# shenyunhang/NA-fWebSOD

Measured on AMD Instinct MI355X. Metric: images/sec (600px, 2000 proposals) VGG16-C5 WSDDN fwd+bwd, higher is better.
Workload: dtype f32 (2xf16 split, 3-pass f16 MFMA, fp32 accumulate)

## Files before the change

na-fwebsod_amd/csrc/misc_ops.hip:

```cpp
#include <float.h>
#include <math.h>
#include "naws_common.h"

thread_local int g_naws_last_hip_error = 0;

extern "C" const char* naws_version(void) { return "naws-hip 0.1 (gfx950)"; }
extern "C" int naws_last_hip_error(void) { return g_naws_last_hip_error; }

#include <atomic>
#include <mutex>
#include <string.h>
namespace {
constexpr int LDS_SLOTS = 512;
constexpr int MAX_DEV = 256;
struct LdsSlot {
  std::atomic<const void*> kernel;
  std::atomic<unsigned long long> dev[MAX_DEV / 64];
};
LdsSlot g_lds_slots[LDS_SLOTS];
std::mutex g_lds_mutex;
std::atomic<int> g_knobs[NAWS_KNOB_COUNT] = {{0}, {0}, {0}, {11}, {0}, {42}, {0}, {0}, {0}};
const char* const g_knob_names[NAWS_KNOB_COUNT] = {"gemm", "x3", "h2", "conv_ring", "conv_bn",
                                                    "roi_nw", "wino", "split", "sgd_wgs"};
}

int naws_allow_lds_impl(const void* kernel, int bytes) {
  int dev = 0;
  if (hipGetDevice(&dev) != hipSuccess) return naws_check_launch();
  const bool in_range = dev >= 0 && dev < MAX_DEV;
  const size_t h0 = ((uintptr_t)kernel >> 4) % LDS_SLOTS;
  if (in_range) {
    size_t h = h0;
    for (int probe = 0; probe < LDS_SLOTS; ++probe, h = (h + 1) % LDS_SLOTS) {
      const void* k = g_lds_slots[h].kernel.load(std::memory_order_acquire);
      if (k == kernel) {
        if ((g_lds_slots[h].dev[dev >> 6].load(std::memory_order_acquire) >> (dev & 63)) & 1ULL)
          return NAWS_OK;
        break;
      }
      if (k == nullptr) break;
    }
  }
  std::lock_guard<std::mutex> lock(g_lds_mutex);
  LdsSlot* slot = nullptr;
  if (in_range) {
    size_t h = h0;
    for (int probe = 0; probe < LDS_SLOTS; ++probe, h = (h + 1) % LDS_SLOTS) {
      const void* k = g_lds_slots[h].kernel.load(std::memory_order_relaxed);
      if (k == kernel) { slot = &g_lds_slots[h]; break; }
      if (k == nullptr) {
        slot = &g_lds_slots[h];
        slot->kernel.store(kernel, std::memory_order_release);
        break;
      }
    }
  }
// ... 676 lines not shown
```

na-fwebsod_amd/csrc/naws_common.h:

```cpp
#pragma once
#include <hip/hip_runtime.h>
#include <stdint.h>
#include <algorithm>
#include "naws.h"

#define NAWS_WAVE 64

extern thread_local int g_naws_last_hip_error;

static inline int naws_check_launch() {
  hipError_t e = hipGetLastError();
  if (e != hipSuccess) {
    g_naws_last_hip_error = (int)e;
    return NAWS_ERR_LAUNCH;
  }
  return NAWS_OK;
}

int naws_allow_lds_impl(const void* kernel, int bytes);
template <typename K>
static inline int naws_allow_lds(K kernel, int bytes = 160 * 1024) {
  return naws_allow_lds_impl(reinterpret_cast<const void*>(kernel), bytes);
}

int naws_wino_col_gemm_impl(int P, int Cout, int Cin, const void* V2, const float* invV,
                            const void* U2, const float* scaleU, float* S, hipStream_t stream);

enum NawsKnob { NAWS_KNOB_GEMM = 0, NAWS_KNOB_X3, NAWS_KNOB_H2, NAWS_KNOB_CONV_RING,
                NAWS_KNOB_CONV_BN, NAWS_KNOB_ROI_NW, NAWS_KNOB_WINO, NAWS_KNOB_SPLIT, NAWS_KNOB_SGD_WGS,
                NAWS_KNOB_COUNT };
int naws_knob(int knob);

#define NAWS_REQUIRE_PTR(p) \
  do {                      \
    if ((p) == nullptr) return NAWS_ERR_NULL; \
  } while (0)

static inline int64_t naws_cdiv(int64_t a, int64_t b) { return (a + b - 1) / b; }

__device__ __forceinline__ float wave_sum(float v) {
#pragma unroll
  for (int o = 32; o > 0; o >>= 1) v += __shfl_xor(v, o, 64);
  return v;
}
__device__ __forceinline__ float wave_max(float v) {
#pragma unroll
  for (int o = 32; o > 0; o >>= 1) v = fmaxf(v, __shfl_xor(v, o, 64));
  return v;
}

__device__ __host__ __forceinline__ uint32_t naws_hash_u32(uint64_t seed, uint64_t idx) {
  uint64_t z = seed + 0x9E3779B97F4A7C15ull * (idx + 1);
  z = (z ^ (z >> 30)) * 0xBF58476D1CE4E5B9ull;
  z = (z ^ (z >> 27)) * 0x94D049BB133111EBull;
  z = z ^ (z >> 31);
  return (uint32_t)(z >> 40);
}
__device__ __host__ __forceinline__ bool naws_keep(uint64_t seed, uint64_t idx, uint32_t thr24) {
  return naws_hash_u32(seed, idx) >= thr24;
}
static inline uint32_t naws_drop_threshold(float ratio) {
  double t = (double)ratio * 16777216.0;
  if (t < 0) t = 0;
// ... 174 lines not shown
```

na-fwebsod_amd/csrc/roi_ops.hip:

```cpp
#include <float.h>
#include <stdlib.h>
#include "naws_common.h"

namespace {

struct RoiBins {
  int batch, start_w, start_h, roi_w, roi_h;
};

__device__ __forceinline__ RoiBins roi_frame(const float* roi, float spatial_scale) {
  RoiBins b;
  b.batch = (int)roi[0];
  int start_w = (int)roundf(roi[1] * spatial_scale);
  int start_h = (int)roundf(roi[2] * spatial_scale);
  int end_w = (int)roundf(roi[3] * spatial_scale);
  int end_h = (int)roundf(roi[4] * spatial_scale);
  b.start_w = start_w;
  b.start_h = start_h;
  b.roi_w = max(end_w - start_w + 1, 1);
  b.roi_h = max(end_h - start_h + 1, 1);
  return b;
}

__device__ __forceinline__ void bin_range(int p, float bin_size, int roi_start, int limit,
// ... 116 lines not shown
          }
          for (; w < we; ++w) {
            const float4 v = *reinterpret_cast<const float4*>(row + (int64_t)w * C);
            NAWS_UPD(v)
          }
#undef NAWS_UPD
        }
      }
      tile[(0 * 64 + lane) * PW + pw] = best.x * scale;
      tile[(1 * 64 + lane) * PW + pw] = best.y * scale;
      tile[(2 * 64 + lane) * PW + pw] = best.z * scale;
      tile[(3 * 64 + lane) * PW + pw] = best.w * scale;
    }
    __syncthreads();
    const int count = nch * PW;
    for (int i = lane; i < count; i += 64) {
      const int cl = i / PW, pw = i - cl * PW;
      Y[obase + (int64_t)cl * nb + ph * PW + pw] = tile[((cl & 3) * 64 + (cl >> 2)) * PW + pw];
    }
    __syncthreads();
  }
}

struct RoiPlaneOut {
  unsigned short* P;
  float* inv_scale;
  const unsigned* amax_words;
  int n_words;
  long long plane;
  int R;
  int bf16;
};

template <bool PLANES, bool HIER = false, int NW = 1, int RG = 1>
__global__ __launch_bounds__(64 * NW) void roi_pool_nhwc_xcd_kernel(
    const float* __restrict__ X, int C, int H, int W, const float* __restrict__ rois, int R,
    const float* __restrict__ boost, int PH, int PW, float spatial_scale, int nslices,
    float* __restrict__ Y, RoiPlaneOut po, const float* __restrict__ M2 = nullptr,
    const float* __restrict__ M4 = nullptr) {
  static_assert(NW % RG == 0, "waves per roi");
  extern __shared__ __attribute__((aligned(16))) char smem_raw[];
  const int nb = PH * PW;
  float* tiles = reinterpret_cast<float*>(smem_raw);
  float* s_scale = tiles + RG * 64 * nb;
  const int slice = blockIdx.x % nslices;
  const int r0 = (blockIdx.x / nslices) * RG;
  const int lane = threadIdx.x & 63;
  const int wave = threadIdx.x >> 6;
  const int q = wave % RG;
  const int r = r0 + q;
  const int cg = lane & 15, g = lane >> 4;
  const int c0 = slice * 64;
  float* tile = tiles + q * 64 * nb;

  if (r < R) {
    const RoiBins rb = roi_frame(rois + (int64_t)r * 5, spatial_scale);
    const float bin_h = (float)rb.roi_h / (float)PH;
    const float bin_w = (float)rb.roi_w / (float)PW;
    const float scale = boost ? boost[r] : 1.0f;
    const int64_t img_off = (int64_t)rb.batch * H * W * C + c0 + cg * 4;
    const float* Xn = X + img_off;
    if constexpr (PLANES) {
      if (wave < RG && lane == 0 && !po.bf16) {
        const float bound =
            __uint_as_float(po.amax_words[min(rb.batch, po.n_words - 1)]) * fabsf(scale);
        float sc, isc;
        naws_f16x2_scales(__float_as_uint(bound), sc, isc);
        s_scale[q] = sc;
        if (slice == 0) po.inv_scale[r] = isc;
      }
    }

    const int pwg = (PW + 3) / 4;
    for (int step = wave / RG; step < PH * pwg; step += NW / RG) {
      const int ph = step / pwg, pw0 = (step - ph * pwg) * 4;
      int hs, he;
      bin_range(ph, bin_h, rb.start_h, H, hs, he);
      const int pw = pw0 + g;
      const bool lane_on = pw < PW;
      int ws = 0, we = 0;
      if (lane_on) bin_range(pw, bin_w, rb.start_w, W, ws, we);
      const bool empty = (he <= hs) || (we <= ws);
      const float init = empty ? 0.0f : -FLT_MAX;
      float4 best = make_float4(init, init, init, init);
#define NAWS_UPD(v) \
  best.x = (v.x > best.x) ? v.x : best.x; best.y = (v.y > best.y) ? v.y : best.y; \
  best.z = (v.z > best.z) ? v.z : best.z; best.w = (v.w > best.w) ? v.w : best.w;
      int hbeg = hs;
      if constexpr (HIER) {
        const int dmin = min(he - hs, we - ws);
        if (dmin >= 2) {
          const int Lb = dmin >= 4 ? 4 : 2;
          const float* S = (dmin >= 4 ? M4 : M2) + img_off;
          const int hl = he - Lb, wl = we - Lb;
          for (int h = hs; h < he; h += 2 * Lb) {
            const float* q0 = S + (int64_t)min(h, hl) * W * C;
            const float* q1 = S + (int64_t)min(h + Lb, hl) * W * C;
            int w = ws;
            for (; w + 2 * Lb < we; w += 2 * Lb) {
              const float4 a0 = *reinterpret_cast<const float4*>(q0 + (int64_t)w * C);
              const float4 a1 = *reinterpret_cast<const float4*>(q0 + (int64_t)(w + Lb) * C);
              const float4 b0 = *reinterpret_cast<const float4*>(q1 + (int64_t)w * C);
              const float4 b1 = *reinterpret_cast<const float4*>(q1 + (int64_t)(w + Lb) * C);
              NAWS_UPD(a0) NAWS_UPD(a1) NAWS_UPD(b0) NAWS_UPD(b1)
            }
            {
              const int w0 = min(w, wl), w1 = min(w + Lb, wl);
              const float4 a0 = *reinterpret_cast<const float4*>(q0 + (int64_t)w0 * C);
              const float4 a1 = *reinterpret_cast<const float4*>(q0 + (int64_t)w1 * C);
              const float4 b0 = *reinterpret_cast<const float4*>(q1 + (int64_t)w0 * C);
              const float4 b1 = *reinterpret_cast<const float4*>(q1 + (int64_t)w1 * C);
              NAWS_UPD(a0) NAWS_UPD(a1) NAWS_UPD(b0) NAWS_UPD(b1)
            }
// ... 20 lines not shown
        }
        for (; w < we; ++w) {
          const float4 a = *reinterpret_cast<const float4*>(q0 + (int64_t)w * C);
          const float4 b = *reinterpret_cast<const float4*>(q1 + (int64_t)w * C);
          NAWS_UPD(a) NAWS_UPD(b)
        }
      }
      for (; h < he; ++h) {
        const float* row = Xn + (int64_t)h * W * C;
        int w = ws;
        for (; w + 4 <= we; w += 4) {
          const float4 v0 = *reinterpret_cast<const float4*>(row + (int64_t)(w + 0) * C);
          const float4 v1 = *reinterpret_cast<const float4*>(row + (int64_t)(w + 1) * C);
          const float4 v2 = *reinterpret_cast<const float4*>(row + (int64_t)(w + 2) * C);
          const float4 v3 = *reinterpret_cast<const float4*>(row + (int64_t)(w + 3) * C);
          NAWS_UPD(v0) NAWS_UPD(v1) NAWS_UPD(v2) NAWS_UPD(v3)
        }
        for (; w < we; ++w) {
          const float4 v = *reinterpret_cast<const float4*>(row + (int64_t)w * C);
          NAWS_UPD(v)
        }
      }
#undef NAWS_UPD
      if (lane_on) {
        const int bin = ph * PW + pw;
        tile[(cg * 4 + 0) * nb + bin] = best.x * scale;
        tile[(cg * 4 + 1) * nb + bin] = best.y * scale;
        tile[(cg * 4 + 2) * nb + bin] = best.z * scale;
        tile[(cg * 4 + 3) * nb + bin] = best.w * scale;
      }
    }
  }
  __syncthreads();
  const int count = 64 * nb;
  if constexpr (!PLANES) {
    for (int i = threadIdx.x; i < RG * count; i += 64 * NW) {
      const int qq = i / count, k = i - qq * count;
      if (r0 + qq < R) Y[((int64_t)(r0 + qq) * C + c0) * nb + k] = tiles[i];
    }
  } else {
    const int slab0 = slice * (count / 16);
    for (int i = threadIdx.x; i < RG * (count / 8); i += 64 * NW) {
      const int hh = i & 1, qq = (i >> 1) % RG, j = i / (2 * RG);
      if (r0 + qq >= R) continue;
      const float* src = tiles + qq * count + j * 16 + hh * 8;
      if (po.bf16) {
        unsigned short q8[8];
#pragma unroll
        for (int e = 0; e < 8; ++e) {
          const __bf16 b = (__bf16)src[e];
          q8[e] = *reinterpret_cast<const unsigned short*>(&b);
        }
        uint4 w;
        w.x = q8[0] | ((unsigned)q8[1] << 16); w.y = q8[2] | ((unsigned)q8[3] << 16);
        w.z = q8[4] | ((unsigned)q8[5] << 16); w.w = q8[6] | ((unsigned)q8[7] << 16);
        *reinterpret_cast<uint4*>(po.P + ((long long)(slab0 + j) * po.R + r0 + qq) * 16 + hh * 8) = w;
        continue;
      }
      const float sc = s_scale[qq];
      unsigned short hi[8], lo[8];
#pragma unroll
      for (int e = 0; e < 8; ++e) {
        const float t = src[e] * sc;
        const _Float16 a = (_Float16)t;
        float rr = t - (float)a;
        if (!(fabsf(t) <= 65504.f)) rr = 0.f;
        const _Float16 b = (_Float16)rr;
        hi[e] = *reinterpret_cast<const unsigned short*>(&a);
        lo[e] = *reinterpret_cast<const unsigned short*>(&b);
      }
      const long long dst = ((long long)(slab0 + j) * po.R + r0 + qq) * 16 + hh * 8;
      uint4 wh, wl;
      wh.x = hi[0] | ((unsigned)hi[1] << 16); wh.y = hi[2] | ((unsigned)hi[3] << 16);
      wh.z = hi[4] | ((unsigned)hi[5] << 16); wh.w = hi[6] | ((unsigned)hi[7] << 16);
// ... 28 lines not shown
  if (k >= K) return;
  const int sl = threadIdx.x >> 4, kk = threadIdx.x & 15;
  unsigned w[8];
#pragma unroll
  for (int i = 0; i < 8; ++i) w[i] = t[sl][2 * i][kk] | ((unsigned)t[sl][2 * i + 1][kk] << 16);
  unsigned short* o = dst + ((long long)blockIdx.y * K + k) * 16;
  *reinterpret_cast<uint4*>(o) = make_uint4(w[0], w[1], w[2], w[3]);
  *reinterpret_cast<uint4*>(o + 8) = make_uint4(w[4], w[5], w[6], w[7]);
}

template <int STEP>
__global__ __launch_bounds__(256) void roi_maxmap_kernel(const float* __restrict__ S, int H, int W,
                                                         int C, float* __restrict__ D,
                                                         long long total4) {
  const long long i = (long long)blockIdx.x * 256 + threadIdx.x;
  if (i >= total4) return;
  const int c4 = C / 4;
  const int cq = (int)(i % c4);
  const long long pix = i / c4;
  const int x = (int)(pix % W), y = (int)((pix / W) % H);
  const int dy = (y + STEP < H) ? STEP : 0, dx = (x + STEP < W) ? STEP : 0;
  const float* base = S + (pix * C + cq * 4);
  const float4 v00 = *reinterpret_cast<const float4*>(base);
  const float4 v01 = *reinterpret_cast<const float4*>(base + (long long)dx * C);
  const float4 v10 = *reinterpret_cast<const float4*>(base + (long long)dy * W * C);
  const float4 v11 = *reinterpret_cast<const float4*>(base + ((long long)dy * W + dx) * C);
  float4 m = make_float4(-FLT_MAX, -FLT_MAX, -FLT_MAX, -FLT_MAX);
#define NAWS_MX(b, v) \
  b.x = (v.x > b.x) ? v.x : b.x; b.y = (v.y > b.y) ? v.y : b.y; \
  b.z = (v.z > b.z) ? v.z : b.z; b.w = (v.w > b.w) ? v.w : b.w;
  NAWS_MX(m, v00) NAWS_MX(m, v01) NAWS_MX(m, v10) NAWS_MX(m, v11)
#undef NAWS_MX
  *reinterpret_cast<float4*>(D + (pix * C + cq * 4)) = m;
}

__global__ void roi_pool_nchw_kernel(int64_t total, const float* __restrict__ X, int C, int H,
                                     int W, const float* __restrict__ rois,
                                     const float* __restrict__ boost, int PH, int PW,
                                     float spatial_scale, float* __restrict__ Y,
                                     int32_t* __restrict__ argmax) {
  for (int64_t idx = (int64_t)blockIdx.x * blockDim.x + threadIdx.x; idx < total;
       idx += (int64_t)gridDim.x * blockDim.x) {
    int pw = (int)(idx % PW);
    int ph = (int)((idx / PW) % PH);
    int c = (int)((idx / PW / PH) % C);
    int r = (int)(idx / PW / PH / C);
    const RoiBins rb = roi_frame(rois + (int64_t)r * 5, spatial_scale);
    const float bin_h = (float)rb.roi_h / (float)PH;
    const float bin_w = (float)rb.roi_w / (float)PW;
    int hs, he, ws, we;
    bin_range(ph, bin_h, rb.start_h, H, hs, he);
    bin_range(pw, bin_w, rb.start_w, W, ws, we);
    const bool empty = (he <= hs) || (we <= ws);
    float best = empty ? 0.0f : -FLT_MAX;
    int besti = -1;
    const float* Xc = X + ((int64_t)rb.batch * C + c) * H * W;
    for (int h = hs; h < he; ++h)
      for (int w = ws; w < we; ++w) {
        float v = Xc[h * W + w];
        if (v > best) { best = v; besti = h * W + w; }
      }
    Y[idx] = best * (boost ? boost[r] : 1.0f);
    if (argmax) argmax[idx] = besti;
  }
}

// ... 76 lines not shown
                       rois, boost, pooled_h, pooled_w, spatial_scale, Y, argmax);
  }
  return naws_check_launch();
}

extern "C" int naws_roi_pool_f_f16x2_fwd(const float* X, int N, int C, int H, int W,
                                         const float* rois, int R, const float* boost,
                                         int pooled_h, int pooled_w, float spatial_scale,
                                         const uint32_t* amax_words, int n_words, void* planes,
                                         float* scales, void* stream) {
  if (R <= 0 || N <= 0 || C <= 0 || H <= 0 || W <= 0 || pooled_h <= 0 || pooled_w <= 0 || n_words <= 0)
    return NAWS_ERR_SHAPE;
  NAWS_REQUIRE_PTR(X); NAWS_REQUIRE_PTR(rois); NAWS_REQUIRE_PTR(amax_words);
  NAWS_REQUIRE_PTR(planes); NAWS_REQUIRE_PTR(scales);
  const long long K = (long long)C * pooled_h * pooled_w;
  if (C % 64 != 0 || pooled_h * pooled_w > 256 || K % 32 != 0 || (int64_t)R * (C / 64) >= 0x7fffffffLL)
    return NAWS_ERR_UNSUPPORTED;
  if ((((uintptr_t)X | (uintptr_t)planes) & 15) != 0) return NAWS_ERR_ARG;
  RoiPlaneOut po;
  po.P = (unsigned short*)planes; po.inv_scale = scales + R; po.amax_words = (const unsigned*)amax_words;
  po.n_words = n_words; po.plane = K * R; po.R = R; po.bf16 = 0;
  hipLaunchKernelGGL(roi_pool_nhwc_xcd_kernel<true>, dim3((unsigned)(R * (C / 64))), dim3(64),
                     (size_t)(64 * pooled_h * pooled_w + 1) * sizeof(float), (hipStream_t)stream, X, C,
                     H, W, rois, R, boost, pooled_h, pooled_w, spatial_scale, C / 64, (float*)nullptr,
                     po);
  return naws_check_launch();
}

extern "C" int64_t naws_roi_pool_workspace_floats(int N, int C, int H, int W) {
  if (N <= 0 || C <= 0 || H <= 0 || W <= 0) return 0;
  return (int64_t)2 * N * H * W * C;
}

static int roi_maxmaps(const float* X, int N, int C, int H, int W, float* M2, float* M4,
                       hipStream_t s) {
  const long long total4 = (long long)N * H * W * (C / 4);
  if (naws_cdiv(total4, 256) > 0x7fffffffLL) return NAWS_ERR_UNSUPPORTED;
  hipLaunchKernelGGL(roi_maxmap_kernel<1>, dim3((unsigned)naws_cdiv(total4, 256)), dim3(256), 0, s, X, H,
                     W, C, M2, total4);
  hipLaunchKernelGGL(roi_maxmap_kernel<2>, dim3((unsigned)naws_cdiv(total4, 256)), dim3(256), 0, s,
                     (const float*)M2, H, W, C, M4, total4);
  return naws_check_launch();
}

extern "C" int naws_roi_pool_f_nhwc_hier_fwd(const float* X, int N, int C, int H, int W,
                                             const float* rois, int R, const float* boost,
                                             int pooled_h, int pooled_w, float spatial_scale,
                                             float* workspace, float* Y, void* stream) {
  if (R < 0 || N <= 0 || C <= 0 || H <= 0 || W <= 0 || pooled_h <= 0 || pooled_w <= 0)
    return NAWS_ERR_SHAPE;
  if (R == 0) return NAWS_OK;
  NAWS_REQUIRE_PTR(X); NAWS_REQUIRE_PTR(rois); NAWS_REQUIRE_PTR(Y); NAWS_REQUIRE_PTR(workspace);
  if (C % 64 != 0 || pooled_h * pooled_w > 256 || (int64_t)R * (C / 64) >= 0x7fffffffLL)
    return NAWS_ERR_UNSUPPORTED;
  if ((((uintptr_t)X | (uintptr_t)workspace) & 15) != 0) return NAWS_ERR_ARG;
  hipStream_t s = (hipStream_t)stream;
  const int rc = roi_maxmaps(X, N, C, H, W, workspace, workspace + (long long)N * H * W * C, s);
  if (rc != NAWS_OK) return rc;
  hipLaunchKernelGGL((roi_pool_nhwc_xcd_kernel<false, true, 4>), dim3((unsigned)(R * (C / 64))), dim3(256),
                     (size_t)(64 * pooled_h * pooled_w + 1) * sizeof(float), s, X, C, H, W, rois, R,
                     boost, pooled_h, pooled_w, spatial_scale, C / 64, Y, RoiPlaneOut{},
                     (const float*)workspace, (const float*)(workspace + (long long)N * H * W * C));
  return naws_check_launch();
}

static int roi_pool_planes_mapped(const float* X, int N, int C, int H, int W, const float* rois,
                                  int R, const float* boost, int pooled_h, int pooled_w,
                                  float spatial_scale, const uint32_t* amax_words, int n_words,
                                  const float* M2, const float* M4, void* planes, float* scales,
                                  hipStream_t s, int bf16 = 0, int R_total = 0, int r_first = 0) {
  const long long K = (long long)C * pooled_h * pooled_w;
  if (R_total <= 0) { R_total = R; r_first = 0; }
  rois += (long long)r_first * 5;
  if (boost) boost += r_first;
  RoiPlaneOut po;
  po.P = (unsigned short*)planes + (long long)r_first * 16;
  po.inv_scale = scales ? scales + R_total + r_first : nullptr;
  po.amax_words = (const unsigned*)amax_words;
  po.n_words = n_words; po.plane = K * R_total; po.R = R_total; po.bf16 = bf16;
  const int nw = naws_knob(NAWS_KNOB_ROI_NW);
  (void)nw;
#define NAWS_ROI_LAUNCH(NWV, RGV)                                                                    \
  hipLaunchKernelGGL((roi_pool_nhwc_xcd_kernel<true, true, NWV, RGV>),                               \
                     dim3((unsigned)(naws_cdiv(R, RGV) * (C / 64))), dim3(64 * NWV),                  \
                     (size_t)(RGV * 64 * pooled_h * pooled_w + RGV) * sizeof(float), s, X, C, H, W,  \
                     rois, R, boost, pooled_h, pooled_w, spatial_scale, C / 64, (float*)nullptr, po, \
                     M2, M4)
#ifdef NAWS_AB
  if (nw == 41) NAWS_ROI_LAUNCH(4, 1);
  else if (nw == 44) NAWS_ROI_LAUNCH(4, 4);
  else if (nw == 82) NAWS_ROI_LAUNCH(8, 2);
  else if (nw == 84) NAWS_ROI_LAUNCH(8, 4);
  else
#endif
  NAWS_ROI_LAUNCH(4, 2);
#undef NAWS_ROI_LAUNCH
  return naws_check_launch();
}

static int roi_pool_planes_check(const float* X, int N, int C, int H, int W, const float* rois, int R,
                                 int pooled_h, int pooled_w, const uint32_t* amax_words, int n_words,
                                 const void* planes, const float* scales) {
  if (R <= 0 || N <= 0 || C <= 0 || H <= 0 || W <= 0 || pooled_h <= 0 || pooled_w <= 0 || n_words <= 0)
    return NAWS_ERR_SHAPE;
  NAWS_REQUIRE_PTR(X); NAWS_REQUIRE_PTR(rois); NAWS_REQUIRE_PTR(amax_words);
  NAWS_REQUIRE_PTR(planes); NAWS_REQUIRE_PTR(scales);
  const long long K = (long long)C * pooled_h * pooled_w;
  if (C % 64 != 0 || pooled_h * pooled_w > 256 || K % 32 != 0 || (int64_t)R * (C / 64) >= 0x7fffffffLL)
    return NAWS_ERR_UNSUPPORTED;
  if ((((uintptr_t)X | (uintptr_t)planes) & 15) != 0) return NAWS_ERR_ARG;
  return NAWS_OK;
}

extern "C" int naws_roi_pool_f_f16x2_hier_fwd(const float* X, int N, int C, int H, int W,
                                              const float* rois, int R, const float* boost,
                                              int pooled_h, int pooled_w, float spatial_scale,
                                              const uint32_t* amax_words, int n_words,
                                              float* workspace, void* planes, float* scales,
                                              void* stream) {
  int rc = roi_pool_planes_check(X, N, C, H, W, rois, R, pooled_h, pooled_w, amax_words, n_words,
                                 planes, scales);
  if (rc != NAWS_OK) return rc;
  NAWS_REQUIRE_PTR(workspace);
  if (((uintptr_t)workspace & 15) != 0) return NAWS_ERR_ARG;
  hipStream_t s = (hipStream_t)stream;
  float* M4 = workspace + (long long)N * H * W * C;
  rc = roi_maxmaps(X, N, C, H, W, workspace, M4, s);
  if (rc != NAWS_OK) return rc;
// ... 357 lines not shown
```

na-fwebsod_amd/naws_hip/lib.py:

```python
import ctypes as C
import os

_HERE = os.path.dirname(os.path.abspath(__file__))
LIB_PATH = os.environ.get('NAWS_LIB') or os.path.join(os.path.dirname(_HERE), 'lib',
                                                       'libnaws_hip.so')
_ENV_KNOBS = {'NAWS_GEMM_VARIANT': 'gemm', 'NAWS_X3_VARIANT': 'x3', 'NAWS_H2_VARIANT': 'h2',
              'NAWS_CONV_RING': 'conv_ring', 'NAWS_CONV_BN': 'conv_bn', 'NAWS_ROI_NW': 'roi_nw',
              'NAWS_WINO_VARIANT': 'wino', 'NAWS_SPLIT': 'split', 'NAWS_SGD_WGS': 'sgd_wgs'}

OK, ERR_SHAPE, ERR_ARG, ERR_NULL, ERR_LAUNCH, ERR_UNSUPPORTED = 0, -1, -2, -3, -4, -5
_ERR_NAMES = {
    ERR_SHAPE: 'NAWS_ERR_SHAPE', ERR_ARG: 'NAWS_ERR_ARG', ERR_NULL: 'NAWS_ERR_NULL',
    ERR_LAUNCH: 'NAWS_ERR_LAUNCH', ERR_UNSUPPORTED: 'NAWS_ERR_UNSUPPORTED',
}
LAYOUT_NCHW, LAYOUT_NHWC = 0, 1
EPI_NONE, EPI_BIAS, EPI_BIAS_RELU, EPI_BIAS_RELU_DROP, EPI_GATE_POS = range(5)
UN_LOG, UN_SCALE, UN_REPLACE_NAN, UN_LEAKY_RELU, UN_CLIP, UN_RELU = range(6)
BIN_ADD, BIN_SUB, BIN_MUL, BIN_DIV, BIN_GATE_POS = range(5)
PLANES_F16X2, PLANES_BF16X3, PLANES_BF16 = range(3)

p, i32, i64, u64, f32 = C.c_void_p, C.c_int, C.c_int64, C.c_uint64, C.c_float

PROTOTYPES = {
    'naws_conv3x3_c3_nchw_to_nhwc_fwd': [p, p, p, i32, i32, i32, i32, i32, p, p],
    'naws_conv3x3_pack_weight': [p, i32, i32, p, p],
    'naws_conv3x3_nhwc_fwd': [p, p, p, i32, i32, i32, i32, i32, i32, i32, p, p],
    'naws_maxpool2x2_nhwc_fwd': [p, i32, i32, i32, i32, i32, p, p],
    'naws_winograd_weight_transform': [p, i32, i32, p, p],
    'naws_conv3x3_winograd_nhwc_fwd': [p, p, p, i32, i32, i32, i32, i32, i32, i32, p, p, p],
    'naws_nchw_to_nhwc': [p, i32, i32, i32, i32, p, p],
    'naws_nhwc_to_nchw': [p, i32, i32, i32, i32, p, p],
    'naws_roi_pool_f_fwd': [p, i32, i32, i32, i32, i32, p, i32, p, i32, i32, f32, p, p, p],
    'naws_roi_context_fwd': [p, i32, f32, i32, i32, p, p, p],
    'naws_roi_loop_pool_fwd': [p, i32, i32, i32, i32, i32, p, i32, p, i32, i32, f32, p, p, p],
    'naws_roi_feature_boost_fwd': [p, p, i32, i32, p, p],
    'naws_roi_feature_boost_bwd': [p, p, i32, i32, p, p],
    'naws_roi_iou_fwd': [p, i32, p, p],
    'naws_gemm_f32': [i32, i32, i32, i32, i32, p, i32, p, i32, p, i32, i32, i64, i64, i64,
                      i32, p, i64, p, i32, f32, f32, u64, i32, p],
    'naws_dropout_mask': [u64, f32, i64, p, p],
    'naws_colsum_f32': [p, i32, i32, i32, p, i32, p],
# ... 81 lines not shown
    'naws_conv3x3_winograd_nhwc_f16x2_fwd': [p, p, p, p, i32, i32, i32, i32, i32, i32, i32, p, p, p, p, p],
    'naws_winograd4_weight_transform': [p, i32, i32, p, p],
    'naws_conv3x3_winograd4_nhwc_f16x2_fwd': [p, p, p, p, i32, i32, i32, i32, i32, i32, i32, p, p, p, p, p],
    'naws_gemm_f32_f16x2_nt_amax': [i32, i32, i32, p, i64, i64, p, p, i64, i64, p, p, i32, i32,
                                    i64, i64, i64, i64, i64, i32, p, i64, p, i32, f32, f32, u64, i32,
                                    p, i32, p, p, p],
    'naws_gemm_f32_f16x2_nt_cols': [i32, i32, i32, p, i64, i64, p, p, i64, i64, p, p, i32, i32, p, f32,
                                    u64, p, i32, p, i32, i32, p],
    'naws_gemm_f32_amax': [i32, i32, i32, i32, i32, p, i32, p, i32, p, i32, i32, i64, i64, i64,
                           i32, p, i64, p, i32, f32, f32, u64, i32, p, i32, p, p, p],
    'naws_split_f16x2_dual': [p, i32, i32, i32, i32, i64, p, p, p, p, p, i32, p, p, i32, p],
    'naws_gemm_f32_f16x2_nt': [i32, i32, i32, p, i64, i64, p, p, i64, i64, p, p, i32, i32,
                               i64, i64, i64, i64, i64, i32, p, i64, p, i32, f32, f32, u64, i32, p],
}
SPECIAL = {
    'naws_version': ([], C.c_char_p),
    'naws_last_hip_error': ([], i32),
    'naws_entropy_gate_workspace_floats': ([i32, i32, i32, i32], i64),
    'naws_winograd_workspace_floats': ([i32, i32, i32, i32, i32, i32], i64),
    'naws_nms_workspace_bytes': ([i32, i32], i64),
    'naws_roi_label_workspace_bytes': ([i32, i32, i32], i64),
    'naws_softmax_with_loss_n_workspace_floats': ([i32], i64),
    'naws_center_loss_workspace_bytes': ([i32, i32, i32], i64),
    'naws_roi_pool_workspace_floats': ([i32, i32, i32, i32], i64),
    'naws_winograd_f32x3_workspace_floats': ([i32, i32, i32, i32, i32, i32], i64),
    'naws_winograd_f16x2_workspace_floats': ([i32, i32, i32, i32, i32, i32], i64),
    'naws_winograd4_f16x2_workspace_floats': ([i32, i32, i32, i32, i32, i32], i64),
    'naws_gemm_f32_splitk_workspace_floats': ([i32, i32, i32, i32], i64),
}
ALL_SYMBOLS = sorted(list(PROTOTYPES) + list(SPECIAL))
AB_PROTOTYPES = {
    'naws_conv3x3_winograd_nhwc_f16x2_col_fwd': [p, p, p, p, i32, i32, i32, i32, i32, i32, i32, p, p, p,
                                                 p, p],
}


class NawsError(RuntimeError):

    def __init__(self, fn, code, hip_error=0):
        self.fn, self.code, self.hip_error = fn, code, hip_error
        msg = '%s failed: %s' % (fn, _ERR_NAMES.get(code, code))
        if code == ERR_LAUNCH:
            msg += ' (hipError %d)' % hip_error
        super(NawsError, self).__init__(msg)


_lib = None


def load():
    global _lib
    if _lib is not None:
        return _lib
    import torch
    if not os.path.exists(LIB_PATH):
        raise ImportError(
            'libnaws_hip.so not found at %s — build it with `make -C na-fwebsod_amd/csrc` '
            '(or __graft_entry__.build()); there is no CPU fallback.' % LIB_PATH)
    lib = C.CDLL(LIB_PATH)
    for name, argtypes in PROTOTYPES.items():
        fn = getattr(lib, name)
        fn.argtypes, fn.restype = argtypes, i32
    for name, (argtypes, restype) in SPECIAL.items():
        fn = getattr(lib, name)
        fn.argtypes, fn.restype = argtypes, restype
    for name, argtypes in AB_PROTOTYPES.items():
# ... 21 lines not shown
```

na-fwebsod_amd/naws_hip/ops.py:

```python
import ctypes as C

import numpy as np
import torch

from . import lib as L

_f32 = torch.float32


def _stream():
    return torch.cuda.current_stream().cuda_stream


def _chk(t, name, dtype=_f32):
    if not isinstance(t, torch.Tensor) or not t.is_cuda:
        raise TypeError('%s must be a HIP device tensor (the naws ops have no CPU path)' % name)
    if t.dtype != dtype:
        raise TypeError('%s must be %s, got %s' % (name, dtype, t.dtype))
    if not t.is_contiguous():
        raise ValueError('%s must be contiguous' % name)
    return t


def _ptr(t):
# ... 129 lines not shown

def roi_loop_pool(x, rois9, pooled_h=7, pooled_w=7, spatial_scale=0.125, boost=None,
                  layout='NCHW', with_argmax=False):
    _chk(x, 'x'); _chk(rois9, 'rois9')
    if rois9.dim() != 2 or rois9.shape[1] != 9:
        raise L.NawsError('naws_roi_loop_pool_fwd', L.ERR_SHAPE)
    if layout == 'NCHW':
        n, c, h, w = x.shape
        lay = L.LAYOUT_NCHW
    elif layout == 'NHWC':
        n, h, w, c = x.shape
        lay = L.LAYOUT_NHWC
    else:
        raise L.NawsError('naws_roi_loop_pool_fwd', L.ERR_ARG)
    r = rois9.shape[0]
    if boost is not None:
        _chk(boost, 'boost')
        assert boost.numel() == r
    y = torch.empty((r, c, pooled_h, pooled_w), device=x.device, dtype=_f32)
    am = torch.empty((r, c, pooled_h, pooled_w), device=x.device, dtype=torch.int32) \
        if with_argmax else None
    L.call('naws_roi_loop_pool_fwd', x.data_ptr(), lay, n, c, h, w, rois9.data_ptr(), r,
           _ptr(boost), pooled_h, pooled_w, float(spatial_scale), y.data_ptr(), _ptr(am), _stream())
    return (y, am) if with_argmax else y


def roi_maxmaps(x, m2, m4):
    _chk(x, 'x'); _chk(m2, 'm2'); _chk(m4, 'm4')
    if m2.shape != x.shape or m4.shape != x.shape or not (x.is_contiguous() and m2.is_contiguous()
                                                          and m4.is_contiguous()):
        raise TypeError('roi_maxmaps: contiguous maps of x\'s shape')
    n, h, w, c = x.shape
    L.call('naws_roi_maxmaps_fwd', x.data_ptr(), n, c, h, w, m2.data_ptr(), m4.data_ptr(), _stream())


def roi_pool_operand(r, k, device):
    return F16x2(torch.empty((2, k // 16, r, 16), device=device, dtype=torch.float16),
                 torch.empty((2, r), device=device, dtype=_f32))


def roi_pool_f_f16x2_range(x, rois, amax_words, out, r0, r1, maps, pooled_h=7, pooled_w=7,
                           spatial_scale=0.125, boost=None):
    _chk(x, 'x'); _chk(rois, 'rois')
    n, h, w, c = x.shape
    r = rois.shape[0]
    m2, m4 = maps
    _chk(m2, 'm2'); _chk(m4, 'm4')
    if boost is not None:
        _chk(boost, 'boost')
        assert boost.numel() == r
    if out.planes.shape != (2, c * pooled_h * pooled_w // 16, r, 16) or m2.shape != x.shape:
        raise L.NawsError('naws_roi_pool_f_f16x2_mapped_range_fwd', L.ERR_SHAPE)
    L.call('naws_roi_pool_f_f16x2_mapped_range_fwd', x.data_ptr(), n, c, h, w, rois.data_ptr(), r,
           int(r0), int(r1 - r0), _ptr(boost), pooled_h, pooled_w, float(spatial_scale),
           amax_words.data_ptr(), amax_words.numel(), m2.data_ptr(), m4.data_ptr(),
           out.planes.data_ptr(), out.scales.data_ptr(), _stream())
    return out


def roi_pool_f_f16x2(x, rois, amax_words, pooled_h=7, pooled_w=7, spatial_scale=0.125, boost=None,
                     hier=True, maps=None):
    _chk(x, 'x'); _chk(rois, 'rois')
    if rois.dim() != 2 or rois.shape[1] != 5:
        raise L.NawsError('naws_roi_pool_f_f16x2_fwd', L.ERR_SHAPE)
    n, h, w, c = x.shape
    r = rois.shape[0]
# ... 1236 lines not shown
```

Measured before the change: 159.9.

## Fuse ROI max-map passes into one LDS-tiled kernel and reorder slice blocks

Replaces the two elementwise max-map launches with a single tiled kernel that loads an input tile with halo into LDS and writes both the 2x2 and the dilated max maps. This removes one launch and the re-read of M2 from global memory. The ROI pool kernel also gains a block-to-slice mapping that interleaves 8 channel slices per round for cache locality. Behind A/B knobs it adds narrower channel slices and a 4-wide store path. The tiled kernel uses a sizeable LDS allocation, which may limit occupancy.

```diff
diff --git a/na-fwebsod_amd/csrc/misc_ops.hip b/na-fwebsod_amd/csrc/misc_ops.hip
--- a/na-fwebsod_amd/csrc/misc_ops.hip
+++ b/na-fwebsod_amd/csrc/misc_ops.hip
@@ -19,9 +19,11 @@
 };
 LdsSlot g_lds_slots[LDS_SLOTS];
 std::mutex g_lds_mutex;
-std::atomic<int> g_knobs[NAWS_KNOB_COUNT] = {{0}, {0}, {0}, {11}, {0}, {42}, {0}, {0}, {0}};
+std::atomic<int> g_knobs[NAWS_KNOB_COUNT] = {{0}, {0}, {0}, {11}, {0}, {42}, {0}, {0}, {0},
+                                           {0}, {0}};
 const char* const g_knob_names[NAWS_KNOB_COUNT] = {"gemm", "x3", "h2", "conv_ring", "conv_bn",
-                                                    "roi_nw", "wino", "split", "sgd_wgs"};
+                                                    "roi_nw", "wino", "split", "sgd_wgs",
+                                                    "roi_cs", "roi_maps"};
 }
 
 int naws_allow_lds_impl(const void* kernel, int bytes) {
diff --git a/na-fwebsod_amd/csrc/naws_common.h b/na-fwebsod_amd/csrc/naws_common.h
--- a/na-fwebsod_amd/csrc/naws_common.h
+++ b/na-fwebsod_amd/csrc/naws_common.h
@@ -28,7 +28,7 @@
 
 enum NawsKnob { NAWS_KNOB_GEMM = 0, NAWS_KNOB_X3, NAWS_KNOB_H2, NAWS_KNOB_CONV_RING,
                 NAWS_KNOB_CONV_BN, NAWS_KNOB_ROI_NW, NAWS_KNOB_WINO, NAWS_KNOB_SPLIT, NAWS_KNOB_SGD_WGS,
-                NAWS_KNOB_COUNT };
+                NAWS_KNOB_ROI_CS, NAWS_KNOB_ROI_MAPS, NAWS_KNOB_COUNT };
 int naws_knob(int knob);
 
 #define NAWS_REQUIRE_PTR(p) \
diff --git a/na-fwebsod_amd/csrc/roi_ops.hip b/na-fwebsod_amd/csrc/roi_ops.hip
--- a/na-fwebsod_amd/csrc/roi_ops.hip
+++ b/na-fwebsod_amd/csrc/roi_ops.hip
@@ -172,7 +172,7 @@
   int bf16;
 };
 
-template <bool PLANES, bool HIER = false, int NW = 1, int RG = 1>
+template <bool PLANES, bool HIER = false, int NW = 1, int RG = 1, int CS = 64, bool ST2 = false>
 __global__ __launch_bounds__(64 * NW) void roi_pool_nhwc_xcd_kernel(
     const float* __restrict__ X, int C, int H, int W, const float* __restrict__ rois, int R,
     const float* __restrict__ boost, int PH, int PW, float spatial_scale, int nslices,
@@ -181,17 +181,35 @@
   static_assert(NW % RG == 0, "waves per roi");
   extern __shared__ __attribute__((aligned(16))) char smem_raw[];
   const int nb = PH * PW;
+  static_assert(CS == 64 || CS == 32 || CS == 16, "slice width");
+  constexpr int QL = CS / 4;
+  constexpr int SLOTS = 256 / CS;
   float* tiles = reinterpret_cast<float*>(smem_raw);
-  float* s_scale = tiles + RG * 64 * nb;
-  const int slice = blockIdx.x % nslices;
-  const int r0 = (blockIdx.x / nslices) * RG;
+  float* s_scale = tiles + RG * CS * nb;
+  int slice, group;
+  {
+    const int ngroups = (int)(gridDim.x / (unsigned)nslices);
+    const int full = nslices / 8;
+    const int per_round = full ? 8 * ngroups : 0;
+    const int round = full ? (int)(blockIdx.x / (unsigned)per_round) : 0;
+    if (round < full) {
+      const int l = (int)blockIdx.x - round * per_round;
+      slice = round * 8 + (l & 7);
+      group = l >> 3;
+    } else {
+      const int l = (int)blockIdx.x - full * per_round, rem = nslices - full * 8;
+      slice = full * 8 + l % rem;
+      group = l / rem;
+    }
+  }
+  const int r0 = group * RG;
   const int lane = threadIdx.x & 63;
   const int wave = threadIdx.x >> 6;
   const int q = wave % RG;
   const int r = r0 + q;
-  const int cg = lane & 15, g = lane >> 4;
-  const int c0 = slice * 64;
-  float* tile = tiles + q * 64 * nb;
+  const int cg = lane % QL, g = lane / QL;
+  const int c0 = slice * CS;
+  float* tile = tiles + q * CS * nb;
 
   if (r < R) {
     const RoiBins rb = roi_frame(rois + (int64_t)r * 5, spatial_scale);
@@ -212,13 +230,22 @@
     }
 
     const int pwg = (PW + 3) / 4;
-    for (int step = wave / RG; step < PH * pwg; step += NW / RG) {
-      const int ph = step / pwg, pw0 = (step - ph * pwg) * 4;
-      int hs, he;
-      bin_range(ph, bin_h, rb.start_h, H, hs, he);
-      const int pw = pw0 + g;
-      const bool lane_on = pw < PW;
-      int ws = 0, we = 0;
+    const int nsteps = CS == 64 ? PH * pwg : (nb + SLOTS - 1) / SLOTS;
+    for (int step = wave / RG; step < nsteps; step += NW / RG) {
+      int ph, pw, hs = 0, he = 0, ws = 0, we = 0;
+      bool lane_on;
+      if constexpr (CS == 64) {
+        ph = step / pwg;
+        pw = (step - ph * pwg) * 4 + g;
+        lane_on = pw < PW;
+        bin_range(ph, bin_h, rb.start_h, H, hs, he);
+      } else {
+        const int bin = step * SLOTS + g;
+        lane_on = bin < nb;
+        ph = bin / PW;
+        pw = bin - ph * PW;
+        if (lane_on) bin_range(ph, bin_h, rb.start_h, H, hs, he);
+      }
       if (lane_on) bin_range(pw, bin_w, rb.start_w, W, ws, we);
       const bool empty = (he <= hs) || (we <= ws);
       const float init = empty ? 0.0f : -FLT_MAX;
@@ -305,7 +332,7 @@
     }
   }
   __syncthreads();
-  const int count = 64 * nb;
+  const int count = CS * nb;
   if constexpr (!PLANES) {
     for (int i = threadIdx.x; i < RG * count; i += 64 * NW) {
       const int qq = i / count, k = i - qq * count;
@@ -313,6 +340,41 @@
     }
   } else {
     const int slab0 = slice * (count / 16);
+    if constexpr (ST2) {
+      for (int i = threadIdx.x; i < RG * (count / 4); i += 64 * NW) {
+        const int u = i & 3, qq = (i >> 2) % RG, j = i / (4 * RG);
+        if (r0 + qq >= R) continue;
+        const float4 v = *reinterpret_cast<const float4*>(tiles + qq * count + j * 16 + u * 4);
+        const float src[4] = {v.x, v.y, v.z, v.w};
+        const long long dst = ((long long)(slab0 + j) * po.R + r0 + qq) * 16 + u * 4;
+        unsigned short hi[4], lo[4];
+        if (po.bf16) {
+#pragma unroll
+          for (int e = 0; e < 4; ++e) {
+            const __bf16 b = (__bf16)src[e];
+            hi[e] = *reinterpret_cast<const unsigned short*>(&b);
+          }
+          *reinterpret_cast<uint2*>(po.P + dst) =
+              make_uint2(hi[0] | ((unsigned)hi[1] << 16), hi[2] | ((unsigned)hi[3] << 16));
+          continue;
+        }
+        const float sc = s_scale[qq];
+#pragma unroll
+        for (int e = 0; e < 4; ++e) {
+          const float t = src[e] * sc;
+          const _Float16 a = (_Float16)t;
+          float rr = t - (float)a;
+          if (!(fabsf(t) <= 65504.f)) rr = 0.f;
+          const _Float16 b = (_Float16)rr;
+          hi[e] = *reinterpret_cast<const unsigned short*>(&a);
+          lo[e] = *reinterpret_cast<const unsigned short*>(&b);
+        }
+        *reinterpret_cast<uint2*>(po.P + dst) =
+            make_uint2(hi[0] | ((unsigned)hi[1] << 16), hi[2] | ((unsigned)hi[3] << 16));
+        *reinterpret_cast<uint2*>(po.P + po.plane + dst) =
+            make_uint2(lo[0] | ((unsigned)lo[1] << 16), lo[2] | ((unsigned)lo[3] << 16));
+      }
+    } else
     for (int i = threadIdx.x; i < RG * (count / 8); i += 64 * NW) {
       const int hh = i & 1, qq = (i >> 1) % RG, j = i / (2 * RG);
       if (r0 + qq >= R) continue;
@@ -407,6 +469,61 @@
   NAWS_MX(m, v00) NAWS_MX(m, v01) NAWS_MX(m, v10) NAWS_MX(m, v11)
 #undef NAWS_MX
   *reinterpret_cast<float4*>(D + (pix * C + cq * 4)) = m;
+}
+
+constexpr int MT_Y = 8, MT_X = 16, MT_CQ = 8;
+__global__ __launch_bounds__(256) void roi_maxmaps_tile_kernel(const float* __restrict__ X, int H, int W,
+                                                               int C, int tiles_x, int tiles_y,
+                                                               int cchunks, float* __restrict__ M2,
+                                                               float* __restrict__ M4) {
+  constexpr int XW = MT_X + 3, XH = MT_Y + 3, MW = MT_X + 2, MH = MT_Y + 2;
+  __shared__ float4 sx[XH * XW][MT_CQ];
+  __shared__ float4 sm[MH * MW][MT_CQ];
+  unsigned b = blockIdx.x;
+  const int cc = (int)(b % (unsigned)cchunks); b /= (unsigned)cchunks;
+  const int tx = (int)(b % (unsigned)tiles_x); b /= (unsigned)tiles_x;
+  const int ty = (int)(b % (unsigned)tiles_y);
+  const int n = (int)(b / (unsigned)tiles_y);
+  const int cq = threadIdx.x % MT_CQ, p = threadIdx.x / MT_CQ;
+  const int c = (cc * MT_CQ + cq) * 4;
+  const bool on = c < C;
+  const int y0 = ty * MT_Y, x0 = tx * MT_X;
+  const long long img = (long long)n * H * W * C + (on ? c : 0);
+#define NAWS_MX(b, v) \
+  b.x = (v.x > b.x) ? v.x : b.x; b.y = (v.y > b.y) ? v.y : b.y; \
+  b.z = (v.z > b.z) ? v.z : b.z; b.w = (v.w > b.w) ? v.w : b.w;
+  if (on)
+    for (int i = p; i < XH * XW; i += 256 / MT_CQ) {
+      const int ly = i / XW, lx = i - ly * XW;
+      const int gy = min(y0 + ly, H - 1), gx = min(x0 + lx, W - 1);
+      sx[i][cq] = *reinterpret_cast<const float4*>(X + img + ((long long)gy * W + gx) * C);
+    }
+  __syncthreads();
+  if (on)
+    for (int i = p; i < MH * MW; i += 256 / MT_CQ) {
+      const int ly = i / MW, lx = i - ly * MW;
+      const float4 v00 = sx[ly * XW + lx][cq], v01 = sx[ly * XW + lx + 1][cq];
+      const float4 v10 = sx[(ly + 1) * XW + lx][cq], v11 = sx[(ly + 1) * XW + lx + 1][cq];
+      float4 m = make_float4(-FLT_MAX, -FLT_MAX, -FLT_MAX, -FLT_MAX);
+      NAWS_MX(m, v00) NAWS_MX(m, v01) NAWS_MX(m, v10) NAWS_MX(m, v11)
+      sm[i][cq] = m;
+      if (ly < MT_Y && lx < MT_X && y0 + ly < H && x0 + lx < W)
+        *reinterpret_cast<float4*>(M2 + img + ((long long)(y0 + ly) * W + x0 + lx) * C) = m;
+    }
+  __syncthreads();
+  if (on)
+    for (int i = p; i < MT_Y * MT_X; i += 256 / MT_CQ) {
+      const int ly = i / MT_X, lx = i - ly * MT_X;
+      const int y = y0 + ly, x = x0 + lx;
+      if (y >= H || x >= W) continue;
+      const int dy = (y + 2 < H) ? 2 : 0, dx = (x + 2 < W) ? 2 : 0;
+      const float4 v00 = sm[ly * MW + lx][cq], v01 = sm[ly * MW + lx + dx][cq];
+      const float4 v10 = sm[(ly + dy) * MW + lx][cq], v11 = sm[(ly + dy) * MW + lx + dx][cq];
+      float4 m = make_float4(-FLT_MAX, -FLT_MAX, -FLT_MAX, -FLT_MAX);
+      NAWS_MX(m, v00) NAWS_MX(m, v01) NAWS_MX(m, v10) NAWS_MX(m, v11)
+      *reinterpret_cast<float4*>(M4 + img + ((long long)y * W + x) * C) = m;
+    }
+#undef NAWS_MX
 }
 
 __global__ void roi_pool_nchw_kernel(int64_t total, const float* __restrict__ X, int C, int H,
@@ -549,14 +666,47 @@
   return (int64_t)2 * N * H * W * C;
 }
 
+#ifdef NAWS_AB
+constexpr long long ROI_L2_BUDGET = 3584LL * 1024;
+static int roi_slice_budget_width(int H, int W) {
+  for (int cs = 64; cs > 16; cs /= 2)
+    if (3LL * H * W * cs * (long long)sizeof(float) <= ROI_L2_BUDGET) return cs;
+  return 16;
+}
+extern "C" int naws_roi_pool_slice_budget_width(int C, int H, int W) {
+  if (C <= 0 || H <= 0 || W <= 0) return NAWS_ERR_SHAPE;
+  if (C % 64 != 0) return NAWS_ERR_UNSUPPORTED;
+  return roi_slice_budget_width(H, W);
+}
+#endif
+static int roi_slice_width_now(int C, int H, int W) {
+#ifdef NAWS_AB
+  const int k = naws_knob(NAWS_KNOB_ROI_CS);
+  if (k == 32 || k == 16) return k;
+  if (k == -1) return roi_slice_budget_width(H, W);
+#endif
+  return 64;
+}
+
 static int roi_maxmaps(const float* X, int N, int C, int H, int W, float* M2, float* M4,
                        hipStream_t s) {
-  const long long total4 = (long long)N * H * W * (C / 4);
-  if (naws_cdiv(total4, 256) > 0x7fffffffLL) return NAWS_ERR_UNSUPPORTED;
-  hipLaunchKernelGGL(roi_maxmap_kernel<1>, dim3((unsigned)naws_cdiv(total4, 256)), dim3(256), 0, s, X, H,
-                     W, C, M2, total4);
-  hipLaunchKernelGGL(roi_maxmap_kernel<2>, dim3((unsigned)naws_cdiv(total4, 256)), dim3(256), 0, s,
-                     (const float*)M2, H, W, C, M4, total4);
+#ifdef NAWS_AB
+  if (naws_knob(NAWS_KNOB_ROI_MAPS) == 1) {
+    const long long total4 = (long long)N * H * W * (C / 4);
+    if (naws_cdiv(total4, 256) > 0x7fffffffLL) return NAWS_ERR_UNSUPPORTED;
+    hipLaunchKernelGGL(roi_maxmap_kernel<1>, dim3((unsigned)naws_cdiv(total4, 256)), dim3(256), 0, s, X,
+                       H, W, C, M2, total4);
+    hipLaunchKernelGGL(roi_maxmap_kernel<2>, dim3((unsigned)naws_cdiv(total4, 256)), dim3(256), 0, s,
+                       (const float*)M2, H, W, C, M4, total4);
+    return naws_check_launch();
+  }
+#endif
+  const int tiles_x = (int)naws_cdiv(W, MT_X), tiles_y = (int)naws_cdiv(H, MT_Y);
+  const int cchunks = (int)naws_cdiv(C, 4 * MT_CQ);
+  const long long blocks = (long long)N * tiles_y * tiles_x * cchunks;
+  if (blocks > 0x7fffffffLL) return NAWS_ERR_UNSUPPORTED;
+  hipLaunchKernelGGL(roi_maxmaps_tile_kernel, dim3((unsigned)blocks), dim3(256), 0, s, X, H, W, C,
+                     tiles_x, tiles_y, cchunks, M2, M4);
   return naws_check_launch();
 }
 
@@ -574,10 +724,21 @@
   hipStream_t s = (hipStream_t)stream;
   const int rc = roi_maxmaps(X, N, C, H, W, workspace, workspace + (long long)N * H * W * C, s);
   if (rc != NAWS_OK) return rc;
-  hipLaunchKernelGGL((roi_pool_nhwc_xcd_kernel<false, true, 4>), dim3((unsigned)(R * (C / 64))), dim3(256),
-                     (size_t)(64 * pooled_h * pooled_w + 1) * sizeof(float), s, X, C, H, W, rois, R,
-                     boost, pooled_h, pooled_w, spatial_scale, C / 64, Y, RoiPlaneOut{},
-                     (const float*)workspace, (const float*)(workspace + (long long)N * H * W * C));
+  const int cs = roi_slice_width_now(C, H, W);
+  if ((int64_t)R * (C / cs) >= 0x7fffffffLL) return NAWS_ERR_UNSUPPORTED;
+#define NAWS_ROI_LAUNCH(CSV)                                                                          \
+  hipLaunchKernelGGL((roi_pool_nhwc_xcd_kernel<false, true, 4, 1, CSV>),                              \
+                     dim3((unsigned)(R * (C / CSV))), dim3(256),                                      \
+                     (size_t)(CSV * pooled_h * pooled_w + 1) * sizeof(float), s, X, C, H, W, rois, R, \
+                     boost, pooled_h, pooled_w, spatial_scale, C / CSV, Y, RoiPlaneOut{},             \
+                     (const float*)workspace, (const float*)(workspace + (long long)N * H * W * C))
+#ifdef NAWS_AB
+  if (cs == 16) NAWS_ROI_LAUNCH(16);
+  else if (cs == 32) NAWS_ROI_LAUNCH(32);
+  else
+#endif
+  NAWS_ROI_LAUNCH(64);
+#undef NAWS_ROI_LAUNCH
   return naws_check_launch();
 }
 
@@ -597,20 +758,31 @@
   po.n_words = n_words; po.plane = K * R_total; po.R = R_total; po.bf16 = bf16;
   const int nw = naws_knob(NAWS_KNOB_ROI_NW);
   (void)nw;
-#define NAWS_ROI_LAUNCH(NWV, RGV)                                                                    \
-  hipLaunchKernelGGL((roi_pool_nhwc_xcd_kernel<true, true, NWV, RGV>),                               \
-                     dim3((unsigned)(naws_cdiv(R, RGV) * (C / 64))), dim3(64 * NWV),                  \
-                     (size_t)(RGV * 64 * pooled_h * pooled_w + RGV) * sizeof(float), s, X, C, H, W,  \
-                     rois, R, boost, pooled_h, pooled_w, spatial_scale, C / 64, (float*)nullptr, po, \
-                     M2, M4)
+  const int cs = roi_slice_width_now(C, H, W);
+  if ((int64_t)R * (C / cs) >= 0x7fffffffLL) return NAWS_ERR_UNSUPPORTED;
+#define NAWS_ROI_LAUNCH(NWV, RGV, CSV, ...)                                                          \
+  hipLaunchKernelGGL((roi_pool_nhwc_xcd_kernel<true, true, NWV, RGV, CSV, ##__VA_ARGS__>),           \
+                     dim3((unsigned)(naws_cdiv(R, RGV) * (C / CSV))), dim3(64 * NWV),                 \
+                     (size_t)(RGV * CSV * pooled_h * pooled_w + RGV) * sizeof(float), s, X, C, H, W, \
+                     rois, R, boost, pooled_h, pooled_w, spatial_scale, C / CSV, (float*)nullptr,    \
+                     po, M2, M4)
 #ifdef NAWS_AB
-  if (nw == 41) NAWS_ROI_LAUNCH(4, 1);
-  else if (nw == 44) NAWS_ROI_LAUNCH(4, 4);
-  else if (nw == 82) NAWS_ROI_LAUNCH(8, 2);
-  else if (nw == 84) NAWS_ROI_LAUNCH(8, 4);
-  else
+#define NAWS_ROI_FORMS(CSV)                          \
+  if (nw == 41) NAWS_ROI_LAUNCH(4, 1, CSV);          \
+  else if (nw == 44) NAWS_ROI_LAUNCH(4, 4, CSV);     \
+  else if (nw == 82) NAWS_ROI_LAUNCH(8, 2, CSV);     \
+  else if (nw == 84) NAWS_ROI_LAUNCH(8, 4, CSV);     \
+  else if (nw == 22) NAWS_ROI_LAUNCH(2, 2, CSV);     \
+  else if (nw == 142) NAWS_ROI_LAUNCH(4, 2, CSV, true);    \
+  else if (nw == 144) NAWS_ROI_LAUNCH(4, 4, CSV, true);   \
+  else NAWS_ROI_LAUNCH(4, 2, CSV)
+  if (cs == 16) { NAWS_ROI_FORMS(16); }
+  else if (cs == 32) { NAWS_ROI_FORMS(32); }
+  else { NAWS_ROI_FORMS(64); }
+#undef NAWS_ROI_FORMS
+#else
+  NAWS_ROI_LAUNCH(4, 2, 64);
 #endif
-  NAWS_ROI_LAUNCH(4, 2);
 #undef NAWS_ROI_LAUNCH
   return naws_check_launch();
 }
diff --git a/na-fwebsod_amd/naws_hip/lib.py b/na-fwebsod_amd/naws_hip/lib.py
--- a/na-fwebsod_amd/naws_hip/lib.py
+++ b/na-fwebsod_amd/naws_hip/lib.py
@@ -6,7 +6,8 @@
                                                        'libnaws_hip.so')
 _ENV_KNOBS = {'NAWS_GEMM_VARIANT': 'gemm', 'NAWS_X3_VARIANT': 'x3', 'NAWS_H2_VARIANT': 'h2',
               'NAWS_CONV_RING': 'conv_ring', 'NAWS_CONV_BN': 'conv_bn', 'NAWS_ROI_NW': 'roi_nw',
-              'NAWS_WINO_VARIANT': 'wino', 'NAWS_SPLIT': 'split', 'NAWS_SGD_WGS': 'sgd_wgs'}
+              'NAWS_WINO_VARIANT': 'wino', 'NAWS_SPLIT': 'split', 'NAWS_SGD_WGS': 'sgd_wgs',
+              'NAWS_ROI_CS': 'roi_cs', 'NAWS_ROI_MAPS': 'roi_maps'}
 
 OK, ERR_SHAPE, ERR_ARG, ERR_NULL, ERR_LAUNCH, ERR_UNSUPPORTED = 0, -1, -2, -3, -4, -5
 _ERR_NAMES = {
@@ -154,6 +155,7 @@
 AB_PROTOTYPES = {
     'naws_conv3x3_winograd_nhwc_f16x2_col_fwd': [p, p, p, p, i32, i32, i32, i32, i32, i32, i32, p, p, p,
                                                  p, p],
+    'naws_roi_pool_slice_budget_width': [i32, i32, i32],
 }
 
 
diff --git a/na-fwebsod_amd/naws_hip/ops.py b/na-fwebsod_amd/naws_hip/ops.py
--- a/na-fwebsod_amd/naws_hip/ops.py
+++ b/na-fwebsod_amd/naws_hip/ops.py
@@ -185,6 +185,13 @@
         raise TypeError('roi_maxmaps: contiguous maps of x\'s shape')
     n, h, w, c = x.shape
     L.call('naws_roi_maxmaps_fwd', x.data_ptr(), n, c, h, w, m2.data_ptr(), m4.data_ptr(), _stream())
+
+
+def roi_pool_slice_budget_width(c, h, w):
+    cs = L.load().naws_roi_pool_slice_budget_width(int(c), int(h), int(w))
+    if cs < 0:
+        raise L.NawsError('naws_roi_pool_slice_budget_width', cs)
+    return cs
 
 
 def roi_pool_operand(r, k, device):
```

Result: no change. 159.6 (-0.1%).
